# skywoodsz/qm_control

Hardware: NVIDIA H100
Metric: mpc_wbc_iters_per_s (higher is better)
Workload: dtype f64

## Files before the change

qm_control_b200/csrc/capi_mpc.inc:

```

extern "C" {

int qmb200_centroidal_state_from_rbd(const qmb200_handle* h, int32_t n, const double* rbd, double* x) {
  if (!h || !rbd || !x) return -1; const DevModel& d = h->hm.dev;
  for (int r = 0; r < n; ++r) {
    const double* s = rbd + (size_t)r * QMB200_RBD; double* o = x + (size_t)r * NX;
    const double z = s[0], y = s[1], xr = s[2];
    const double sz = sin(z), cz = cos(z), sy = sin(y), cy = cos(y), sx = sin(xr), cx = cos(xr);
    const double R[9] = {cz * cy, cz * sy * sx - sz * cx, cz * sy * cx + sz * sx, sz * cy, sz * sy * sx + cz * cx, sz * sy * cx - cz * sx, -sy, cy * sx, cy * cx};
    const double w[3] = {s[NQ], s[NQ + 1], s[NQ + 2]};
    const double ed[3] = {(cz * sy / cy) * w[0] + (sy * sz / cy) * w[1] + w[2], -sz * w[0] + cz * w[1], (cz / cy) * w[0] + (sz / cy) * w[1]};
    double c[3]; for (int i = 0; i < 3; ++i) c[i] = R[3 * i] * d.c_nom[0] + R[3 * i + 1] * d.c_nom[1] + R[3 * i + 2] * d.c_nom[2];
    const double cw[3] = {c[1] * w[2] - c[2] * w[1], c[2] * w[0] - c[0] * w[2], c[0] * w[1] - c[1] * w[0]};
    double Rtw[3], IRtw[3], L[3];
    for (int i = 0; i < 3; ++i) Rtw[i] = R[i] * w[0] + R[3 + i] * w[1] + R[6 + i] * w[2];
    for (int i = 0; i < 3; ++i) IRtw[i] = d.I_nom[3 * i] * Rtw[0] + d.I_nom[3 * i + 1] * Rtw[1] + d.I_nom[3 * i + 2] * Rtw[2];
    for (int i = 0; i < 3; ++i) L[i] = R[3 * i] * IRtw[0] + R[3 * i + 1] * IRtw[1] + R[3 * i + 2] * IRtw[2];
    (void)ed;
    for (int i = 0; i < 3; ++i) { o[i] = s[NQ + 3 + i] + cw[i]; o[3 + i] = L[i] / d.total_mass; o[6 + i] = s[3 + i]; o[9 + i] = s[i]; }
    for (int j = 0; j < NJ; ++j) o[12 + j] = s[6 + j];
  }
  return 0;
}

// ... 218 lines not shown
int qmb200_set_pipeline(qmb200_handle* h, int chunks) {
  if (!h) return -1; QMB_CUDA(h, cudaSetDevice(h->device));
  if (chunks < 1 || chunks > qmb200_handle::MAX_CHUNKS) return fail(h, "qmb200_set_pipeline: chunks must be in [1, 8]");
  if (chunks > h->B) chunks = h->B;
  if (!h->fork_ev) QMB_CUDA(h, cudaEventCreateWithFlags(&h->fork_ev, cudaEventDisableTiming));
  for (int c = 0; c < chunks; ++c) { if (!h->cs[c]) QMB_CUDA(h, cudaStreamCreateWithFlags(&h->cs[c], cudaStreamNonBlocking)); if (!h->join_ev[c]) QMB_CUDA(h, cudaEventCreateWithFlags(&h->join_ev[c], cudaEventDisableTiming)); }
  h->chunks = chunks; return 0;
}
int qmb200_set_profiling(qmb200_handle* h, int on) {
  if (!h) return -1; QMB_CUDA(h, cudaSetDevice(h->device));
  if (on && !h->ev[0]) for (int i = 0; i < 8; ++i) QMB_CUDA(h, cudaEventCreate(&h->ev[i]));
  h->profiling = on != 0; for (double& v : h->kernel_ms) v = 0.0; h->kernel_calls = 0; h->ev_pending = false; return 0;
}
int qmb200_collect_kernel_times(qmb200_handle* h) {
  if (!h || !h->profiling || !h->ev_pending) return -1; QMB_CUDA(h, cudaSetDevice(h->device)); QMB_CUDA(h, cudaEventSynchronize(h->ev[6]));
  const int a[6] = {0, 1, 2, 3, 4, 5}, b[6] = {1, 2, 3, 4, 5, 6};
  for (int i = 0; i < 6; ++i) { float ms = 0; QMB_CUDA(h, cudaEventElapsedTime(&ms, h->ev[a[i]], h->ev[b[i]])); h->kernel_ms[i] += ms; }
  { float ms = 0; QMB_CUDA(h, cudaEventElapsedTime(&ms, h->ev[1], h->ev[7])); h->kernel_ms[6] += ms; }
  h->kernel_calls += 1; h->ev_pending = false; return 0;
}
int qmb200_get_kernel_times(qmb200_handle* h, double* ms6) { if (!h || !ms6) return -1; for (int i = 0; i < 6; ++i) ms6[i] = h->kernel_calls ? h->kernel_ms[i] / h->kernel_calls : 0.0; return 0; }
int qmb200_get_flow_kernel_time(qmb200_handle* h, double* ms) { if (!h || !ms) return -1; *ms = h->kernel_calls ? h->kernel_ms[6] / h->kernel_calls : 0.0; return 0; }
int qmb200_measure_fp64_peak(qmb200_handle* h, double* tflops) { if (!h || !tflops) return -1; QMB_CUDA(h, cudaSetDevice(h->device)); *tflops = measure_fp64_peak(h->stream); QMB_CUDA(h, cudaGetLastError()); return 0; }

int qmb200_debug_get_step(qmb200_handle* h, double* dx , double* du , double* robot ) {
  if (!h) return -1; QMB_CUDA(h, cudaSetDevice(h->device)); const size_t Bn = (size_t)h->B * h->nmax;
  if (dx) QMB_CUDA(h, cudaMemcpy(dx, h->mpc.dx, Bn * NX * 8, cudaMemcpyDeviceToHost)); if (du) QMB_CUDA(h, cudaMemcpy(du, h->mpc.du, Bn * NU * 8, cudaMemcpyDeviceToHost));
  if (robot) QMB_CUDA(h, cudaMemcpy(robot, h->mpc.robot, (size_t)h->B * ROBOT_DBL * 8, cudaMemcpyDeviceToHost)); return 0;
}

}
```

qm_control_b200/csrc/kernels/mpc_api.cuh:

```cuda
#pragma once
#include <cuda_runtime.h>

#include <string>
#include <vector>

#include "dev_common.cuh"

namespace qmb {

constexpr int EMAX = 32, KMAX = 4, TARGET_DIM = 37;
constexpr int LDX = 36, LDB = 28, LDG = 34, LDH = 24;
constexpr int ST_AR = 0;
constexpr int ST_BR = ST_AR + 9 * LDX;
constexpr int ST_Q = ST_BR + 9 * LDB;
constexpr int Q_PACKED = 480;
__host__ __device__ constexpr int q_row_offset(int r) { return (r & 1) ? 2 * ((r >> 1) + 1) * ((r >> 1) + 1) : 2 * (r >> 1) * ((r >> 1) + 1); }
__host__ __device__ constexpr int q_row_padded(int r) { return (r + 2) & ~1; }
static_assert(q_row_offset(29) + q_row_padded(29) == Q_PACKED && q_row_offset(1) == 2 && q_row_offset(2) == 4 && q_row_offset(3) == 8, "packed lower triangle with even rows");
constexpr int ST_TAIL = ST_Q + Q_PACKED;
constexpr int T_PXJ = 0;
constexpr int T_b = 144, T_q = 174, T_r = 204;
constexpr int T_RT = 222;
constexpr int T_SJ = 276;
constexpr int T_PU2 = 372, T_PED = 380;
// ... 7 lines not shown

struct MpcSolutionDev { int32_t* n_nodes = nullptr; double* t = nullptr; int32_t* event = nullptr; double* x = nullptr; double* u = nullptr; };

struct MpcBuffers {
  int B = 0, nmax = 0, cur = 0;
  double *t0 = nullptr, *x0 = nullptr, *event_times = nullptr, *target_times = nullptr, *target_states = nullptr;
  int32_t *n_events = nullptr, *modes = nullptr, *n_target = nullptr;
  MpcSolutionDev sol[2];
  double *ddp_trial = nullptr;
  double *node_rec = nullptr;
  double *stage = nullptr, *gains = nullptr, *dx = nullptr, *du = nullptr, *robot = nullptr, *step_info = nullptr;
  int32_t *stage_i = nullptr, *status = nullptr;
};
bool mpc_alloc(MpcBuffers& m, int B, int nmax, std::string& err, std::vector<void*>& allocs, cudaStream_t stream);
int mpc_configure_device();

struct MpcProblemDev { const double* t0; const double* x0; const int32_t* n_events; const double* event_times; const int32_t* modes; const int32_t* n_target; const double* target_times; const double* target_states; };

int mpc_solve_launch(const DevModel* mdl, const DevModel& host_mdl, MpcBuffers& m, const MpcProblemDev& p, int b0, int b1, cudaStream_t stream, cudaEvent_t* ev = nullptr);
double measure_fp64_peak(cudaStream_t stream);
int mpc_policy_eval_launch(const MpcBuffers& m, const double* t, double* x_des, double* u_des, int32_t* mode, cudaStream_t stream, int b0 = 0, int b1 = -1);
int mpc_fixup_launch(const MpcBuffers& m, cudaStream_t stream);

}
```

qm_control_b200/csrc/kernels/mpc_kernels.cu:

```cuda
#include <cstdlib>
#include "mpc_api.cuh"
#include "mpc_device.cuh"
#include "node_eval.cuh"
#include "wlinalg.cuh"

namespace qmb {

#ifndef QMB_LQ_WARPS
#define QMB_LQ_WARPS 4
#endif
#ifndef QMB_LQ_MINB
#define QMB_LQ_MINB 4
#endif
constexpr int LQ_WARPS = QMB_LQ_WARPS, LS_WARPS = 4, SETUP_WARPS = 4;
enum { MST_ITER_CAP = 1, MST_OVERFLOW = 2, MST_NAN = 4, MST_NOT_PD = 8, MST_NO_STEP = 16, MST_CONVERGED = 32, MST_NEG_DT = 64 };

__device__ __forceinline__ double interval_start(double t, int ev) { return ev == 2 ? t + WEAK_EPS : t; }
__device__ __forceinline__ double interval_end(double t, int ev) { return ev == 1 ? t - WEAK_EPS : t; }
__device__ __forceinline__ int clamp_events(int ne) { return ne < 0 ? 0 : (ne > EMAX ? EMAX : ne); }
__device__ __forceinline__ int clamp_targets(int nk) { return nk < 1 ? 1 : (nk > KMAX ? KMAX : nk); }
__device__ __forceinline__ int flag_mask(int mode) { int m = 0; for (int i = 0; i < 4; ++i) if (contact_flag(mode, i)) m |= 1 << i; return m; }

struct SetupIdx { int iu, ix; double au, ax; };
__host__ __device__ inline size_t setup_smem_per_warp(int nmax) { return (size_t)nmax * (8 + 8 + 4 + sizeof(SetupIdx) + 4) + 8 * EMAX + 64; }
// ... 391 lines not shown
  if (lane < MU) si[SI_FREE + lane] = (lane < m) ? sm.free_idx[lane] : -1;
  if (lane == 0) { si[SI_TYPE] = 0; si[SI_M] = m; si[SI_NDEP] = ndep; tl[T_MISC] = dtw; tl[T_MISC + 1] = dt * cost_val; tl[T_MISC + 2] = dt * dyn_ss; tl[T_MISC + 3] = dt * eq_ss; }
}

#ifndef QMB_TMA
#define QMB_TMA 1
#endif
constexpr int RIC_THREADS = 128, RIC_NTYPE = 512;
struct RicSmem {
  double P[NX * LDX];
  double A[NX * LDX];
  double W[NX * LDX];
  double Bm[NX * LDB], PB[NX * LDB];
  double G[MU * LDG];
  double H[MU * LDH];
  double Lt[MU * MU];
  alignas(16) double tail[TAIL_DBL];
  double dx[32], dut[32], tmp[32];
  double red[RIC_THREADS / 32][4];
  alignas(8) unsigned long long bar[4];
  int flag; int pad_;
  signed char srow[MU + 2], sfirst[MU + 2];
  unsigned char ntype[RIC_NTYPE];
};
static_assert(sizeof(RicSmem) <= 57344 - 64, "Riccati kernel must keep four CTAs per SM");

__device__ __forceinline__ unsigned smem_u32(const void* p) { return (unsigned)__cvta_generic_to_shared(p); }
__device__ __forceinline__ void mbar_init(unsigned long long* b, unsigned count) { asm volatile("mbarrier.init.shared::cta.b64 [%0], %1;\n" ::"r"(smem_u32(b)), "r"(count) : "memory"); }
__device__ __forceinline__ void mbar_expect_tx(unsigned long long* b, unsigned bytes) { asm volatile("mbarrier.arrive.expect_tx.shared::cta.b64 _, [%0], %1;\n" ::"r"(smem_u32(b)), "r"(bytes) : "memory"); }
__device__ __forceinline__ void mbar_wait(unsigned long long* b, unsigned parity) {
  asm volatile("{\n .reg .pred p;\n WAIT_LOOP:\n mbarrier.try_wait.parity.shared::cta.b64 p, [%0], %1;\n @p bra WAIT_DONE;\n bra WAIT_LOOP;\n WAIT_DONE:\n}\n" ::"r"(smem_u32(b)), "r"(parity) : "memory");
}
__device__ __forceinline__ void bulk_g2s(void* dst, const void* src, unsigned bytes, unsigned long long* bar) {
  asm volatile("cp.async.bulk.shared::cluster.global.mbarrier::complete_tx::bytes [%0], [%1], %2, [%3];\n" ::"r"(smem_u32(dst)), "l"(src), "r"(bytes), "r"(smem_u32(bar)) : "memory");
}
__device__ __forceinline__ void cp_async16(void* smem_dst, const void* gmem_src) { asm volatile("cp.async.cg.shared.global [%0], [%1], 16;\n" ::"r"(smem_u32(smem_dst)), "l"(gmem_src) : "memory"); }
__device__ __forceinline__ void cp_async_wait_all() { asm volatile("cp.async.wait_all;\n" ::: "memory"); }
struct CopyGroup {
  unsigned long long* bar; unsigned phase;
  __device__ __forceinline__ void begin(unsigned bytes, int tid) { if (QMB_TMA && tid == 0) mbar_expect_tx(bar, bytes); }
  __device__ __forceinline__ void copy(void* dst, const void* src, unsigned bytes, int tid, int nthr = RIC_THREADS, int t0 = 0) {
    if (QMB_TMA) { if (tid == 0) bulk_g2s(dst, src, bytes, bar); }
    else { const int me = tid - t0; if (me >= 0 && me < nthr) for (unsigned o = 16u * me; o < bytes; o += 16u * nthr) cp_async16((char*)dst + o, (const char*)src + o); }
  }
  __device__ __forceinline__ void wait() { if (QMB_TMA) mbar_wait(bar, phase & 1u); else { cp_async_wait_all(); __syncthreads(); } ++phase; }
  __device__ __forceinline__ void skip() { ++phase; }
};

// ... 32 lines not shown
    for (int n = 0; n < NT; ++n) { const int ri = i0 + 8 * m + g; if (ri < rows) *reinterpret_cast<double2*>(M + ri * ld + j0 + 8 * n + 2 * t) = make_double2(c[m][n][0], c[m][n][1]); }
}
__device__ __forceinline__ int sup_pos(int j, int first) { return j < 6 ? j : ((j >= 9 && j < 12) ? j - 3 : (((unsigned)(j - 12 - first) < 3u) ? 9 + j - 12 - first : -1)); }

__global__ void __launch_bounds__(RIC_THREADS, 4) mpc_riccati_kernel(const DevModel* __restrict__ mdl, int b0, int B, int nmax, MpcProblemDev p, MpcSolutionDev sol, const double* __restrict__ stage,
                                                                  double* __restrict__ gains, double* __restrict__ dxo, double* __restrict__ duo, double* __restrict__ robot, int32_t* __restrict__ status) {
  extern __shared__ __align__(16) unsigned char smem_raw[];
  RicSmem& sm = *reinterpret_cast<RicSmem*>(smem_raw);
  const int tid = threadIdx.x, warp = tid >> 5, lane = tid & 31, ti = tid >> 2, jb = tid & 3; const int b = b0 + blockIdx.x;
  if (status[b] & MST_CONVERGED) return;
  const int n = sol.n_nodes[b]; const int N = n - 1;
  const double* sgb = stage + (size_t)b * nmax * STAGE_DBL; double* gb = gains + (size_t)b * nmax * GAIN_DBL;
  const int lfp = pack_leg_foot(mdl); const double imass = 1.0 / mdl->total_mass;
  for (int e = tid; e < (int)(sizeof(RicSmem) / 8); e += RIC_THREADS) reinterpret_cast<double*>(&sm)[e] = 0.0;
  __syncthreads();
  if (tid < NX && (tid < 3 || tid >= 24)) sm.A[tid * LDX + tid] = 1.0;
  if (tid == 0) { for (int i = 0; i < 4; ++i) mbar_init(&sm.bar[i], 1); asm volatile("fence.mbarrier_init.release.cluster;\n" ::: "memory"); }
  asm volatile("fence.proxy.async.shared::cta;\n" ::: "memory");
  const bool types_in_smem = n <= RIC_NTYPE;
  auto rec_type = [&](int k) -> int { return reinterpret_cast<const int32_t*>(sgb + (size_t)k * STAGE_DBL + ST_TAIL + T_INT)[SI_TYPE]; };
  if (types_in_smem) for (int k = tid; k < n; k += RIC_THREADS) sm.ntype[k] = (unsigned char)rec_type(k);
  auto node_type = [&](int k) -> int { return types_in_smem ? (int)sm.ntype[k] : rec_type(k); };
  CopyGroup gAB{&sm.bar[0], 0u}, gT{&sm.bar[1], 0u}, gQ{&sm.bar[2], 0u}, gF1{&sm.bar[3], 0u};
  auto issue_ab = [&](int k) { const double* sg = sgb + (size_t)k * STAGE_DBL; gAB.begin((9 * LDX + 9 * LDB) * 8, tid);
    gAB.copy(sm.A + 3 * LDX, sg + ST_AR, 9 * LDX * 8, tid); gAB.copy(sm.Bm + 3 * LDB, sg + ST_BR, 9 * LDB * 8, tid); };
  auto issue_tail = [&](int k) { gT.begin(TAIL_DBL * 8, tid); gT.copy(sm.tail, sgb + (size_t)k * STAGE_DBL + ST_TAIL, TAIL_DBL * 8, tid); };
  auto issue_q = [&](int k) { gQ.begin(Q_PACKED * 8, tid); gQ.copy(sm.Bm, sgb + (size_t)k * STAGE_DBL + ST_Q, Q_PACKED * 8, tid); };
  auto expand = [&]() {
    const double* tl = sm.tail; const int32_t* si = reinterpret_cast<const int32_t*>(tl + T_INT); const double dtw = tl[T_MISC];
    for (int e = tid; e < 144; e += RIC_THREADS) { const int j12 = e / 12, c = e - 12 * j12; const int col = sup_col(c, 3 * (j12 / 3));
      sm.A[(12 + j12) * LDX + col] = ((col == 12 + j12) ? 1.0 : 0.0) + dtw * tl[T_PXJ + e]; }
    if (tid < NX && (tid < 3 || tid >= 12)) sm.A[tid * LDX + NX] = tl[T_b + tid];
    for (int e = tid; e < 21 * MU; e += RIC_THREADS) {
      const int rr = e / MU, a = e - rr * MU; const int r = rr < 3 ? rr : rr + 9; const int fa = si[SI_FREE + a]; double v = 0.0;
      if (fa >= 0) {
        if (r < 3) { if (fa < 12 && fa - 3 * (fa / 3) == r) v = dtw * imass; }
        else if (fa == r) v = dtw;
        else if (fa >= 12 && fa < 24) { const int j = fa - 12, lg = j / 3, foot = (lfp >> (2 * lg)) & 3; const int pv = si[SI_PIV + foot];
          if (pv >= 0 && r == 12 + 3 * lg + pv) { const int jf = j - 3 * lg; v = dtw * tl[T_PU2 + 2 * foot + (jf > pv ? jf - 1 : jf)]; } }
      }
      sm.Bm[r * LDB + a] = v;
    }
    if (tid < MU) { const int fa = si[SI_FREE + tid]; int slot = -1, first = 0;
      if (fa >= 12 && fa < 24) { const int j = fa - 12, lg = j / 3, foot = (lfp >> (2 * lg)) & 3; const int pv = si[SI_PIV + foot]; if (pv >= 0) { const int jf = j - 3 * lg; slot = 2 * foot + (jf > pv ? jf - 1 : jf); first = 3 * lg; } }
      sm.srow[tid] = (signed char)slot; sm.sfirst[tid] = (signed char)first; }
  };
  for (int e = tid; e < NX * NX; e += RIC_THREADS) { const int r = e / NX, c = e - r * NX; sm.P[r * LDX + c] = sgb[(size_t)N * STAGE_DBL + ST_Q + q_row_offset(r > c ? r : c) + (r > c ? c : r)]; }
  if (tid < NX) sm.P[tid * LDX + NX] = sgb[(size_t)N * STAGE_DBL + ST_TAIL + T_q + tid];
  double perf0 = 0, perf1 = 0, perf2 = 0;
  for (int k = tid; k < n; k += RIC_THREADS) { const double* pf = sgb + (size_t)k * STAGE_DBL + ST_TAIL + T_MISC + 1; perf0 += pf[0]; perf1 += pf[1]; perf2 += pf[2]; }
  if (tid < NX) { const double d = p.x0[(size_t)b * NX + tid] - sol.x[(size_t)b * nmax * NX + tid]; sm.dx[tid] = d; perf1 += d * d; }
  perf0 = warp_sum(perf0); perf1 = warp_sum(perf1); perf2 = warp_sum(perf2);
  if (lane == 0) { sm.red[warp][0] = perf0; sm.red[warp][1] = perf1; sm.red[warp][2] = perf2; }
  __syncthreads();
  double perf[3]; for (int i = 0; i < 3; ++i) perf[i] = sm.red[0][i] + sm.red[1][i] + sm.red[2][i] + sm.red[3][i];
  if (N >= 1) { issue_tail(N - 1); if (node_type(N - 1) != 1) issue_ab(N - 1); gT.wait(); if (node_type(N - 1) != 1) expand(); }
  int st = 0;
  const int g = lane >> 2, t = lane & 3;
  for (int k = N - 1; k >= 0; --k) {
    const int type = node_type(k); const int tnext = k > 0 ? node_type(k - 1) : 1;
    if (type == 1) {
      __syncthreads();
      if (tid < NX) { double sv = sm.P[tid * LDX + NX]; for (int j = 0; j < NX; ++j) sv = fma(sm.P[tid * LDX + j], sm.tail[T_b + j], sv); sm.tmp[tid] = sv; }
      __syncthreads();
      if (tid < NX) sm.P[tid * LDX + NX] = sm.tmp[tid];
      if (k > 0) { issue_tail(k - 1); if (tnext != 1) issue_ab(k - 1); gT.wait(); if (tnext != 1) expand(); }
      continue;
    }
    gAB.wait(); if (QMB_TMA) __syncthreads();
    const double dtw_k = sm.tail[T_MISC]; const int acol0 = reinterpret_cast<const int32_t*>(sm.tail + T_INT)[SI_M] - 6;
    { const int i0 = 16 * (warp >> 1), j0 = 16 * (warp & 1);
      double c[2][2][2] = {};
      if (warp & 1) {
#pragma unroll
        for (int m = 0; m < 2; ++m) { const int ri = i0 + 8 * m + g; if (ri < NX) {
            if (t < 3) { c[m][1][0] = sm.P[(24 + 2 * t) * LDX + ri]; c[m][1][1] = sm.P[(25 + 2 * t) * LDX + ri]; }
            else { double sv = sm.P[ri * LDX + NX];
#pragma unroll
              for (int kk = 24; kk < NX; ++kk) sv = fma(sm.P[kk * LDX + ri], sm.A[kk * LDX + NX], sv);
              c[m][1][0] = sv; } } } }
      warp_mma<24, 2, 2, false>(sm.P, LDX, i0, sm.A, LDX, j0, c, g, t);
      cfrag_store<2, 2>(sm.W, LDX, i0, j0, NX, c, g, t);
      double d[1][3][2];
#pragma unroll
      for (int nn = 0; nn < 3; ++nn)
#pragma unroll
        for (int e = 0; e < 2; ++e) { const int a = 8 * nn + 2 * t + e - acol0, ri = 8 * warp + g; d[0][nn][e] = ((unsigned)a < 6u && ri < NX) ? dtw_k * sm.P[(24 + a) * LDX + ri] : 0.0; }
      warp_mma<24, 1, 3, false>(sm.P, LDX, 8 * warp, sm.Bm, LDB, 0, d, g, t);
      cfrag_store<1, 3>(sm.PB, LDB, 8 * warp, 0, NX, d, g, t); }
    __syncthreads();
    if (tid < NX) sm.P[tid * LDX + NX] = sm.tail[T_q + tid];
    { const double* tl = sm.tail; const int32_t* si = reinterpret_cast<const int32_t*>(tl + T_INT); const int mm = si[SI_M];
      double c[3][1][2];
#pragma unroll
      for (int mt = 0; mt < 3; ++mt) { const int a = 8 * mt + g; const bool rowok = a < MU; const int slot = rowok ? sm.srow[a] : -1, first = rowok ? sm.sfirst[a] : 0;
#pragma unroll
        for (int e = 0; e < 2; ++e) { const int j = 8 * warp + 2 * t + e; double v = 0.0;
          if (rowok) { if (j == NX) v = tl[T_r + a]; else if (slot >= 0 && j < NX) { const int ps = sup_pos(j, first); if (ps >= 0) v = tl[T_SJ + slot * 12 + ps]; }
            if ((unsigned)(a - acol0) < 6u) v = fma(dtw_k, sm.W[(24 + a - acol0) * LDX + j], v); }
          c[mt][0][e] = v; } }
      warp_mma<24, 3, 1, false>(sm.Bm, LDB, 0, sm.W, LDX, 8 * warp, c, g, t); cfrag_store<3, 1>(sm.G, LDG, 0, 8 * warp, MU, c, g, t);
      if (warp < 3) { double d[3][1][2];
#pragma unroll
        for (int mt = 0; mt < 3; ++mt) { const int a = 8 * mt + g; const int fa = (a < MU) ? si[SI_FREE + a] : -1;
#pragma unroll
          for (int e = 0; e < 2; ++e) { const int cc = 8 * warp + 2 * t + e; double v = 0.0;
            if (a < MU && cc < MU) { if (a >= mm) v = (a == cc) ? 1.0 : 0.0;
              else if (fa >= 24) v = (a == cc) ? tl[T_RT + 3 * a] : 0.0;
              else { const int fc = si[SI_FREE + cc]; if (fc >= 0 && fc / 3 == fa / 3) v = tl[T_RT + 3 * a + fc - 3 * (fc / 3)]; }
              if ((unsigned)(a - acol0) < 6u) v = fma(dtw_k, sm.PB[(24 + a - acol0) * LDB + cc], v); }
            d[mt][0][e] = v; } }
        warp_mma<24, 3, 1, false>(sm.Bm, LDB, 0, sm.PB, LDB, 8 * warp, d, g, t); cfrag_store<3, 1>(sm.H, LDH, 0, 8 * warp, MU, d, g, t); } }
    __syncthreads();
    issue_q(k);
    if (k > 0) issue_tail(k - 1);
    const int sw = (k + b) & 3;
    if (!QMB_TMA) gQ.wait();
    if (warp == sw) {
      if (QMB_TMA) gQ.skip();
      double hr[MU], y[MU]; double dinv = 0.0; bool ok = true; double* Yb = sm.PB;
#pragma unroll
      for (int c = 0; c < MU; ++c) { hr[c] = (lane < MU) ? sm.H[c * LDH + lane] : 0.0; y[c] = sm.G[c * LDG + lane]; }
#pragma unroll
      for (int j = 0; j < MU; ++j) {
        const double djj = __shfl_sync(FULL, hr[j], j); if (!(djj > 0.0)) ok = false;
        const double inv = rsqrt(djj); const double lij = hr[j] * inv;
        if (lane == j) dinv = inv;
        if (lane < MU) sm.Lt[j * MU + lane] = lij;
        y[j] *= inv; Yb[j * LDX + lane] = y[j];
#pragma unroll
        for (int c = j + 1; c < MU; ++c) { const double lcj = __shfl_sync(FULL, lij, c); hr[c] = fma(-lij, lcj, hr[c]); y[c] = fma(-lcj, y[j], y[c]); }
      }
      if (lane < MU) sm.dut[lane] = dinv;
      if (!ok && lane == 0) sm.flag = 1;
      __syncwarp();
      double* gk = gb + (size_t)k * GAIN_DBL;
#pragma unroll
      for (int a = MU - 1; a >= 0; --a) {
        asm volatile("" ::: "memory");
        y[a] *= sm.dut[a];
        gk[a * LDG + lane] = -y[a];
#pragma unroll
        for (int c = 0; c < a; ++c) y[c] = fma(-sm.Lt[c * MU + a], y[a], y[c]);
      }
    } else {
      if (QMB_TMA) gQ.wait();
      const int hi = (warp - sw - 1) & 3;
      for (int tile = hi; tile < 16; tile += 3) { const int i0 = 8 * (tile >> 2), j0 = 8 * (tile & 3);
        double c[1][1][2]; const int ri = i0 + g;
#pragma unroll
        for (int e = 0; e < 2; ++e) { const int cj = j0 + 2 * t + e; double v = (ri < NX && cj <= NX) ? (cj == NX ? sm.P[ri * LDX + NX] : (cj <= ri ? sm.Bm[q_row_offset(ri) + cj] : sm.Bm[q_row_offset(cj) + ri])) : 0.0;
          if (ri >= 24 && ri < NX && cj <= NX) v += sm.W[ri * LDX + cj];
          c[0][0][e] = v; }
        warp_mma<24, 1, 1, false>(sm.A, LDX, i0, sm.W, LDX, j0, c, g, t); cfrag_store<1, 1>(sm.P, LDX, i0, j0, NX, c, g, t); }
    }
    __syncthreads();
    if (sm.flag) { st |= MST_NOT_PD; if (k > 0) gT.wait(); break; }
    if (k > 0) { if (tnext != 1) issue_ab(k - 1); gT.wait(); if (tnext != 1) expand(); }
    { const double* Yb = sm.PB; const int i0 = 16 * (warp >> 1), j0 = 16 * (warp & 1);
      double c[2][2][2]; cfrag_load<2, 2>(sm.P, LDX, i0, j0, NX, c, g, t); warp_mma<MU, 2, 2, true>(Yb, LDX, i0, Yb, LDX, j0, c, g, t); cfrag_store<2, 2>(sm.P, LDX, i0, j0, NX, c, g, t); }
  }
  __syncthreads();
  double armijo = 0.0, dxn2 = 0.0, dun2 = 0.0;
  if (!(st & MST_NOT_PD)) {
    auto issue_fwd = [&](int k) {
      if (k >= N) return; const int o = k & 1; CopyGroup& cg = o ? gF1 : gAB; const double* sg = sgb + (size_t)k * STAGE_DBL; const bool ev = node_type(k) == 1;
      cg.begin((ev ? 0 : (GAIN_DBL + 9 * LDX + 9 * LDB) * 8) + TAIL_DBL * 8, tid);
      cg.copy((o ? sm.P : sm.A) + 9 * LDX, sg + ST_TAIL, TAIL_DBL * 8, tid);
      if (!ev) { cg.copy(o ? sm.W : sm.G, gb + (size_t)k * GAIN_DBL, GAIN_DBL * 8, tid); cg.copy(o ? sm.P : sm.A, sg + ST_AR, 9 * LDX * 8, tid); cg.copy(o ? sm.PB : sm.Bm, sg + ST_BR, 9 * LDB * 8, tid); } };
    issue_fwd(0);
    for (int k = 0; k < N; ++k) {
      const int o = k & 1; const double* Kb = o ? sm.W : sm.G; const double* ARb = o ? sm.P : sm.A; const double* BRb = o ? sm.PB : sm.Bm; const double* tl = (o ? sm.P : sm.A) + 9 * LDX;
      double* dxk = dxo + ((size_t)b * nmax + k) * NX; double* duk = duo + ((size_t)b * nmax + k) * NU;
      const double* dxc = (k & 1) ? sm.tmp : sm.dx; double* dxn = (k & 1) ? sm.dx : sm.tmp;
      if (o) gF1.wait(); else gAB.wait();
      if (QMB_TMA) __syncthreads();
      issue_fwd(k + 1);
      const int32_t* si = reinterpret_cast<const int32_t*>(tl + T_INT); const int type = si[SI_TYPE], ndep = si[SI_NDEP], mm = si[SI_M]; const double dtw = tl[T_MISC];
      if (tid < NX) { const double dxi = dxc[tid]; dxk[tid] = dxi; dxn2 += dxi * dxi; }
      if (type == 1) { if (tid < NX) { duk[tid] = 0.0; dxn[tid] = dxc[tid] + tl[T_b + tid]; } continue; }
      { double s = 0.0;
        if (ti < MU) { const double* kr = Kb + ti * LDG + jb * 8; const double* dx = dxc + jb * 8;
#pragma unroll
          for (int v = 0; v < 8; ++v) s = fma(kr[v], dx[v], s); }
        s += __shfl_xor_sync(FULL, s, 1); s += __shfl_xor_sync(FULL, s, 2); if (ti < MU && jb == 0) sm.dut[ti] = s + Kb[ti * LDG + NX]; }
// ... 1 lines not shown
      {
        static_assert(MAXDEP * 8 == RIC_THREADS, "one 8-thread group per dependent input");
        const int d = tid >> 3, q8 = tid & 7; double s = 0.0; const int di = (d < ndep) ? si[SI_DEP + d] : -1;
        if (di >= 12) { const int j = di - 12, lg = j / 3, first = 3 * lg; const double* px = tl + T_PXJ + j * 12;
          s = px[q8] * dxc[sup_col(q8, first)]; if (q8 < 4) s = fma(px[q8 + 8], dxc[sup_col(q8 + 8, first)], s);
          if (q8 >= 4 && q8 < 6) { const int foot = (lfp >> (2 * lg)) & 3; const int col = si[SI_PCOL + 2 * foot + q8 - 4]; if (si[SI_PIV + foot] >= 0 && col >= 0) s = fma(tl[T_PU2 + 2 * foot + q8 - 4], sm.dut[col], s); } }
        s += __shfl_xor_sync(FULL, s, 1); s += __shfl_xor_sync(FULL, s, 2); s += __shfl_xor_sync(FULL, s, 4);
        if (di >= 0 && q8 == 0) { const double full = s + tl[T_PED + d]; duk[di] = full; dun2 += full * full; if (di >= 12) dxn[di] = dxc[di] + dtw * s + tl[T_b + di]; } }
      if (tid < NX) armijo += tl[T_q + tid] * dxc[tid];
      if (tid < MU) { const double dut = sm.dut[tid]; armijo += tl[T_r + tid] * dut; const int fi = si[SI_FREE + tid];
        if (fi >= 0) { duk[fi] = dut; dun2 += dut * dut; if (fi >= 12) dxn[fi] = dxc[fi] + dtw * dut + tl[T_b + fi]; } }
      if (warp == 1 && lane < 3) { double acc = 0.0; for (int a = 0; a < mm; ++a) { const int fa = si[SI_FREE + a]; if (fa < 12 && fa - 3 * (fa / 3) == lane) acc += sm.dut[a]; }
        dxn[lane] = dxc[lane] + dtw * imass * acc + tl[T_b + lane]; }
      if (warp >= 2) { const int rr = (tid - 64) >> 2; double s = 0.0;
        if (rr < 9) { const double* ar = ARb + rr * LDX + jb * 8; const double* dx = dxc + jb * 8;
#pragma unroll
          for (int v = 0; v < 8; ++v) s = fma(ar[v], dx[v], s);
          if (jb < 3) { const double* br = BRb + rr * LDB + jb * 8; const double* du = sm.dut + jb * 8;
#pragma unroll
            for (int v = 0; v < 8; ++v) s = fma(br[v], du[v], s); } }
        s += __shfl_xor_sync(FULL, s, 1); s += __shfl_xor_sync(FULL, s, 2); if (rr < 9 && jb == 0) dxn[3 + rr] = s + tl[T_b + 3 + rr]; }
    }
    __syncthreads();
    if (tid < NX) { const double dxi = ((N & 1) ? sm.tmp : sm.dx)[tid]; dxo[((size_t)b * nmax + N) * NX + tid] = dxi; duo[((size_t)b * nmax + N) * NU + tid] = 0.0; dxn2 += dxi * dxi; armijo += sgb[(size_t)N * STAGE_DBL + ST_TAIL + T_q + tid] * dxi; }
  }
  armijo = warp_sum(armijo); dxn2 = warp_sum(dxn2); dun2 = warp_sum(dun2);
  __syncthreads();
  if (lane == 0) { sm.red[warp][0] = armijo; sm.red[warp][1] = dxn2; sm.red[warp][2] = dun2; }
  __syncthreads();
  if (tid == 0) { double a = 0, x2 = 0, u2 = 0; for (int w = 0; w < RIC_THREADS / 32; ++w) { a += sm.red[w][0]; x2 += sm.red[w][1]; u2 += sm.red[w][2]; }
    double* rb = robot + (size_t)b * ROBOT_DBL; rb[0] = a; rb[1] = perf[0]; rb[2] = perf[1]; rb[3] = perf[2]; rb[4] = sqrt(x2); rb[5] = sqrt(u2); if (st) atomicOr(&status[b], st); }
}

__device__ __forceinline__ void fixup_inputs(MpcSolutionDev sol, int b, int nmax, int n, int tid, int nthreads) {
  const int32_t* ge = sol.event + (size_t)b * nmax; double* gu = sol.u + (size_t)b * nmax * NU;
  for (int i = tid; i < NU; i += nthreads) for (int k = 1; k < n; ++k) if ((k == n - 1) || (ge[k] == 1)) gu[(size_t)k * NU + i] = gu[(size_t)(k - 1) * NU + i];
}

#ifndef QMB_LS_MINB
#define QMB_LS_MINB 4
#endif
__global__ void __launch_bounds__(32 * LS_WARPS, QMB_LS_MINB) mpc_linesearch_kernel(const DevModel* __restrict__ mdl, int b0, int B, int nmax, MpcProblemDev p, MpcSolutionDev sol, const double* __restrict__ dxo, const double* __restrict__ duo,
                                                                     const double* __restrict__ robot, int32_t* __restrict__ status, double* __restrict__ step_info, int iteration) {
  __shared__ double red[LS_WARPS][3]; __shared__ int decision; __shared__ double s_ev[EMAX]; __shared__ unsigned char s_modes[EMAX + 8];
  const int tid = threadIdx.x, warp = tid >> 5, lane = tid & 31; const int b = b0 + blockIdx.x; if (b >= B) return;
  if (status[b] & MST_CONVERGED) return;
  const int n = sol.n_nodes[b]; const int N = n - 1;
  const double* gt = sol.t + (size_t)b * nmax; const int32_t* ge = sol.event + (size_t)b * nmax;
  double* gx = sol.x + (size_t)b * nmax * NX; double* gu = sol.u + (size_t)b * nmax * NU; const double* gdx = dxo + (size_t)b * nmax * NX; const double* gdu = duo + (size_t)b * nmax * NU;
// ... 279 lines not shown
  for (int it = 0; it < iters; ++it) {
    mpc_flow_kernel<<<(unsigned)((nodes + 32 * FL_WARPS - 1) / (32 * FL_WARPS)), 32 * FL_WARPS, FL_SMEM, stream>>>(mdl, b0, b1, nmax, p, next, m.node_rec, m.status);
    if (ev && it == iters - 1) cudaEventRecord(ev[7], stream);
    mpc_lq_kernel<<<(unsigned)((nodes + LQ_WARPS - 1) / LQ_WARPS), 32 * LQ_WARPS, sizeof(LqSmem) * LQ_WARPS, stream>>>(mdl, b0, b1, nmax, p, next, m.node_rec, m.stage, m.status);
    if (ev && it == iters - 1) cudaEventRecord(ev[2], stream);
    mpc_riccati_kernel<<<nb, RIC_THREADS, sizeof(RicSmem), stream>>>(mdl, b0, b1, nmax, p, next, m.stage, m.gains, m.dx, m.du, m.robot, m.status);
    if (ev && it == iters - 1) cudaEventRecord(ev[3], stream);
    if (ddp) { mpc_rollout_trials_kernel<<<(nb + ro_rpc - 1) / ro_rpc, ro_rpc * tr_pitch, (size_t)ro_rpc * GAIN_DBL * 8, stream>>>(mdl, b0, b1, nmax, p, next, m.stage, m.gains, m.ddp_trial, m.robot, m.status, n_trials, tr_pitch, ro_rpc);
      mpc_rollout_kernel<<<ro_grid, RO_THREADS, 0, stream>>>(mdl, b0, b1, nmax, p, next, m.stage, m.gains, m.ddp_trial, m.robot, m.status, m.step_info, 2, n_trials, tr_pitch, it); ++launched; }
    else mpc_linesearch_kernel<<<nb, 32 * LS_WARPS, 0, stream>>>(mdl, b0, b1, nmax, p, next, m.dx, m.du, m.robot, m.status, m.step_info, it);
    launched += 4;
  }
  if (ev) cudaEventRecord(ev[4], stream);
  return launched;
}

int mpc_policy_eval_launch(const MpcBuffers& m, const double* t, double* x_des, double* u_des, int32_t* mode, cudaStream_t stream, int b0, int b1) {
  if (b1 < 0) b1 = m.B; if (b1 <= b0) return 0;
  mpc_policy_eval_kernel<<<(b1 - b0 + 3) / 4, 128, 0, stream>>>(b0, b1, m.nmax, m.sol[m.cur], m.n_events, m.event_times, m.modes, t, x_des, u_des, mode);
  return 1;
}
int mpc_fixup_launch(const MpcBuffers& m, cudaStream_t stream) { mpc_fixup_kernel<<<m.B, 32, 0, stream>>>(m.B, m.nmax, m.sol[m.cur]); return 1; }

__global__ void __launch_bounds__(256) fp64_peak_kernel(double* out, int iters, double a, double b) {
  double x0 = threadIdx.x, x1 = x0 + 1, x2 = x0 + 2, x3 = x0 + 3, x4 = x0 + 4, x5 = x0 + 5, x6 = x0 + 6, x7 = x0 + 7;
  for (int i = 0; i < iters; ++i) { x0 = fma(x0, a, b); x1 = fma(x1, a, b); x2 = fma(x2, a, b); x3 = fma(x3, a, b); x4 = fma(x4, a, b); x5 = fma(x5, a, b); x6 = fma(x6, a, b); x7 = fma(x7, a, b); }
  if (x0 + x1 + x2 + x3 + x4 + x5 + x6 + x7 == 12345.678) out[0] = x0;
}
double measure_fp64_peak(cudaStream_t stream) {
  double* d = nullptr; cudaMalloc(&d, 8); cudaEvent_t e0, e1; cudaEventCreate(&e0); cudaEventCreate(&e1);
  int dev = 0, sms = 132; cudaGetDevice(&dev); cudaDeviceGetAttribute(&sms, cudaDevAttrMultiProcessorCount, dev);
  const int blocks = sms * 8, iters = 1 << 15; double best = 0.0;
  fp64_peak_kernel<<<blocks, 256, 0, stream>>>(d, 1024, 0.999999, 1e-9);
  for (int rep = 0; rep < 3; ++rep) {
    cudaEventRecord(e0, stream); fp64_peak_kernel<<<blocks, 256, 0, stream>>>(d, iters, 0.999999, 1e-9); cudaEventRecord(e1, stream); cudaEventSynchronize(e1);
    float ms = 0; cudaEventElapsedTime(&ms, e0, e1); const double tf = 2.0 * 8.0 * iters * 256.0 * blocks / (ms * 1e-3) / 1e12; if (tf > best) best = tf;
  }
  cudaEventDestroy(e0); cudaEventDestroy(e1); cudaFree(d); return best;
}

}
```

qm_control_b200/interface.py:

```python
import ctypes as C
import os

import numpy as np

from . import _lib
from ._lib import NX, NU, RBD, CMD, TARGET, EMAX, KMAX, Config, QmbError, dp, ip


class QMInterface:
    def __init__(self, taskFile=None, urdfFile=None, referenceFile=None, wbcGainsFile=None):
        self.taskFile = taskFile or _lib.asset("qm_task.info")
        self.urdfFile = urdfFile or _lib.asset("qm_robot.urdf")
        self.referenceFile = referenceFile or _lib.asset("qm_reference.info")
        self.gaitFile = _lib.asset("qm_gait.info")
        self.wbcGainsFile = wbcGainsFile
        for what, path in (("Task file", self.taskFile), ("URDF file", self.urdfFile), ("targetCommand file", self.referenceFile)):
            if not os.path.exists(path):
                raise ValueError("[QMInterface] %s not found: %s" % (what, path))


def _f64(a, shape=None):
    a = np.ascontiguousarray(a, dtype=np.float64)
    if shape is not None and tuple(a.shape) != tuple(shape):
        raise ValueError("expected shape %s, got %s" % (shape, a.shape))
# ... 181 lines not shown
        rc = self.lib.qmb200_gait_bin_permutation(n, _p(_f64(prob["t0"])), _p(_i32(prob["n_events"])), _p(_f64(prob["event_times"])), _p(_i32(prob["modes"])), _p(perm))
        if rc != 0:
            raise QmbError("qmb200_gait_bin_permutation failed")
        return perm

    def set_pipeline(self, chunks):
        self._chk(self.lib.qmb200_set_pipeline(self.h, int(chunks)), "qmb200_set_pipeline")

    def set_profiling(self, on=True):
        self._chk(self.lib.qmb200_set_profiling(self.h, 1 if on else 0), "qmb200_set_profiling")

    def collect_kernel_times(self):
        self.lib.qmb200_collect_kernel_times(self.h)

    def kernel_times(self):
        ms = np.zeros(6); self._chk(self.lib.qmb200_get_kernel_times(self.h, _p(ms)), "qmb200_get_kernel_times")
        d = dict(zip(("setup", "lq", "riccati", "linesearch", "policy_eval", "wbc"), ms.tolist()))
        v = C.c_double(); self._chk(self.lib.qmb200_get_flow_kernel_time(self.h, C.byref(v)), "qmb200_get_flow_kernel_time"); d["lq_flow"] = v.value
        return d

    def measure_fp64_peak(self):
        v = C.c_double(); self._chk(self.lib.qmb200_measure_fp64_peak(self.h, C.byref(v)), "qmb200_measure_fp64_peak"); return v.value

    def debug_get_step(self):
        B, N = self.batch, self.nmax; dx = np.zeros((B, N, NX)); du = np.zeros((B, N, NU)); robot = np.zeros((B, 8))
        self._chk(self.lib.qmb200_debug_get_step(self.h, _p(dx), _p(du), _p(robot)), "qmb200_debug_get_step"); return dx, du, robot

    def observation_update(self, rbd, period, t_obs, x_obs):
        B = self.batch; rbd = _f64(rbd, (B, RBD)); period = _f64(period, (B,)); t = _f64(t_obs, (B,)).copy(); x = _f64(x_obs, (B, NX)).copy()
        self._chk(self.lib.qmb200_observation_update(self.h, _p(rbd), _p(period), _p(t), _p(x)), "qmb200_observation_update"); return t, x

    def target_trajectories(self, kind, cmd, t_obs, x_obs, ee_state, last_ee_target):
        B = self.batch; c = np.zeros((B, 7)); cmd = np.asarray(cmd, dtype=np.float64).reshape(B, -1); c[:, :cmd.shape[1]] = cmd
        t = _f64(t_obs, (B,)); x = _f64(x_obs, (B, NX)); ee = _f64(ee_state, (B, 7)); le = _f64(last_ee_target, (B, 7)).copy()
        nt = np.zeros(B, dtype=np.int32); tt = np.zeros((B, KMAX)); ts = np.zeros((B, KMAX, TARGET))
        self._chk(self.lib.qmb200_target_trajectories(self.h, int(kind), _p(c), _p(t), _p(x), _p(ee), _p(le), _p(nt), _p(tt), _p(ts)), "qmb200_target_trajectories"); return nt, tt, ts, le

    def initial_ee_target(self):
        v = np.zeros(7); self.lib.qmb200_initial_ee_target(_p(v)); return np.tile(v, (self.batch, 1))

    def set_arm_gains(self, kp, kd):
        self._chk(self.lib.qmb200_set_arm_gains(self.h, float(kp), float(kd)), "qmb200_set_arm_gains")

    def control_law(self, x_des, u_des, wbc_cmd, t_obs, x_obs, joint_cmd, arm_pos_cmd, last_time):
        B = self.batch; jc = _f64(joint_cmd, (B, 18, 5)).copy(); ap = _f64(arm_pos_cmd, (B, 6)).copy(); lt = _f64(last_time, (B,)).copy(); st = np.zeros(B, dtype=np.int32)
        self._chk(self.lib.qmb200_control_law(self.h, _p(_f64(x_des, (B, NX))), _p(_f64(u_des, (B, NU))), _p(_f64(wbc_cmd, (B, CMD))), _p(_f64(t_obs, (B,))), _p(_f64(x_obs, (B, NX))), _p(jc), _p(ap), _p(lt), _p(st)),
# ... 54 lines not shown
```

Baseline: 19.37.

## Overlap next-stage A/B load and expansion with serial Cholesky in Riccati

In the TMA path, the three helper warps now synchronise on a named barrier after their phase-3 work. They then issue the next node's A/B copy and run the tail expansion, all while the designated warp runs the serial factorisation, rather than doing this after the block-wide barrier. The serial warp waits on the tail copy itself. This aims to hide per-node load and expand latency in the backward Riccati sweep, at the cost of a more intricate sync order and a changed abort path on non-PD. Optional clock64 per-phase profiling counters are also added behind a compile flag, off by default.

```diff
diff --git a/qm_control_b200/csrc/capi_mpc.inc b/qm_control_b200/csrc/capi_mpc.inc
--- a/qm_control_b200/csrc/capi_mpc.inc
+++ b/qm_control_b200/csrc/capi_mpc.inc
@@ -264,6 +264,12 @@
 int qmb200_get_kernel_times(qmb200_handle* h, double* ms6) { if (!h || !ms6) return -1; for (int i = 0; i < 6; ++i) ms6[i] = h->kernel_calls ? h->kernel_ms[i] / h->kernel_calls : 0.0; return 0; }
 int qmb200_get_flow_kernel_time(qmb200_handle* h, double* ms) { if (!h || !ms) return -1; *ms = h->kernel_calls ? h->kernel_ms[6] / h->kernel_calls : 0.0; return 0; }
 int qmb200_measure_fp64_peak(qmb200_handle* h, double* tflops) { if (!h || !tflops) return -1; QMB_CUDA(h, cudaSetDevice(h->device)); *tflops = measure_fp64_peak(h->stream); QMB_CUDA(h, cudaGetLastError()); return 0; }
+#if QMB_RIC_PROF
+int qmb200_ric_profile(qmb200_handle* h, unsigned long long* counters, int n, int reset) {
+  if (!h || !counters) return -1; QMB_CUDA(h, cudaSetDevice(h->device)); QMB_CUDA(h, cudaStreamSynchronize(h->stream));
+  const int got = ric_prof_read(counters, n, reset != 0); if (got < 0) return fail(h, "qmb200_ric_profile: counter copy failed"); return got;
+}
+#endif
 
 int qmb200_debug_get_step(qmb200_handle* h, double* dx , double* du , double* robot ) {
   if (!h) return -1; QMB_CUDA(h, cudaSetDevice(h->device)); const size_t Bn = (size_t)h->B * h->nmax;
diff --git a/qm_control_b200/csrc/kernels/mpc_api.cuh b/qm_control_b200/csrc/kernels/mpc_api.cuh
--- a/qm_control_b200/csrc/kernels/mpc_api.cuh
+++ b/qm_control_b200/csrc/kernels/mpc_api.cuh
@@ -53,4 +53,12 @@
 int mpc_policy_eval_launch(const MpcBuffers& m, const double* t, double* x_des, double* u_des, int32_t* mode, cudaStream_t stream, int b0 = 0, int b1 = -1);
 int mpc_fixup_launch(const MpcBuffers& m, cudaStream_t stream);
 
+#ifndef QMB_RIC_PROF
+#define QMB_RIC_PROF 0
+#endif
+enum RicProfSlot { RP_WAIT = 0, RP_PH1, RP_PH2, RP_PH3_SERIAL, RP_PH3_HELPER, RP_PH3_BARRIER, RP_TAIL, RP_PH4, RP_FWD, RP_NODES, RP_CTAS, RP_NSLOT };
+#if QMB_RIC_PROF
+int ric_prof_read(unsigned long long* out, int n, bool reset);
+#endif
+
 }
diff --git a/qm_control_b200/csrc/kernels/mpc_kernels.cu b/qm_control_b200/csrc/kernels/mpc_kernels.cu
--- a/qm_control_b200/csrc/kernels/mpc_kernels.cu
+++ b/qm_control_b200/csrc/kernels/mpc_kernels.cu
@@ -437,8 +437,26 @@
   int flag; int pad_;
   signed char srow[MU + 2], sfirst[MU + 2];
   unsigned char ntype[RIC_NTYPE];
+#if QMB_RIC_PROF
+  unsigned long long prof[RIC_THREADS / 32][RP_NSLOT];
+#endif
 };
 static_assert(sizeof(RicSmem) <= 57344 - 64, "Riccati kernel must keep four CTAs per SM");
+
+#if QMB_RIC_PROF
+__device__ unsigned long long g_ric_prof[RP_NSLOT];
+#define RIC_PROF_START long long ric_t0 = clock64()
+#define RIC_MARK(s) do { if (lane == 0) { const long long ric_now = clock64(); sm.prof[warp][(s)] += (unsigned long long)(ric_now - ric_t0); ric_t0 = ric_now; } } while (0)
+#define RIC_SKIP() do { if (lane == 0) ric_t0 = clock64(); } while (0)
+#define RIC_COUNT(s) do { if (lane == 0) sm.prof[warp][(s)] += 1ull; } while (0)
+#define RIC_PROF_FLUSH() do { if (lane == 0) for (int s_ = 0; s_ < RP_NSLOT; ++s_) atomicAdd(&g_ric_prof[s_], sm.prof[warp][s_]); } while (0)
+#else
+#define RIC_PROF_START
+#define RIC_MARK(s) ((void)0)
+#define RIC_SKIP() ((void)0)
+#define RIC_COUNT(s) ((void)0)
+#define RIC_PROF_FLUSH() ((void)0)
+#endif
 
 __device__ __forceinline__ unsigned smem_u32(const void* p) { return (unsigned)__cvta_generic_to_shared(p); }
 __device__ __forceinline__ void mbar_init(unsigned long long* b, unsigned count) { asm volatile("mbarrier.init.shared::cta.b64 [%0], %1;\n" ::"r"(smem_u32(b)), "r"(count) : "memory"); }
@@ -517,16 +535,17 @@
   if (types_in_smem) for (int k = tid; k < n; k += RIC_THREADS) sm.ntype[k] = (unsigned char)rec_type(k);
   auto node_type = [&](int k) -> int { return types_in_smem ? (int)sm.ntype[k] : rec_type(k); };
   CopyGroup gAB{&sm.bar[0], 0u}, gT{&sm.bar[1], 0u}, gQ{&sm.bar[2], 0u}, gF1{&sm.bar[3], 0u};
-  auto issue_ab = [&](int k) { const double* sg = sgb + (size_t)k * STAGE_DBL; gAB.begin((9 * LDX + 9 * LDB) * 8, tid);
-    gAB.copy(sm.A + 3 * LDX, sg + ST_AR, 9 * LDX * 8, tid); gAB.copy(sm.Bm + 3 * LDB, sg + ST_BR, 9 * LDB * 8, tid); };
+  auto issue_ab = [&](int k, int me = -1) { if (me < 0) me = tid; const double* sg = sgb + (size_t)k * STAGE_DBL; gAB.begin((9 * LDX + 9 * LDB) * 8, me);
+    gAB.copy(sm.A + 3 * LDX, sg + ST_AR, 9 * LDX * 8, me); gAB.copy(sm.Bm + 3 * LDB, sg + ST_BR, 9 * LDB * 8, me); };
   auto issue_tail = [&](int k) { gT.begin(TAIL_DBL * 8, tid); gT.copy(sm.tail, sgb + (size_t)k * STAGE_DBL + ST_TAIL, TAIL_DBL * 8, tid); };
   auto issue_q = [&](int k) { gQ.begin(Q_PACKED * 8, tid); gQ.copy(sm.Bm, sgb + (size_t)k * STAGE_DBL + ST_Q, Q_PACKED * 8, tid); };
-  auto expand = [&]() {
+  auto expand = [&](int me = -1, int nthr = RIC_THREADS) {
+    if (me < 0) me = tid;
     const double* tl = sm.tail; const int32_t* si = reinterpret_cast<const int32_t*>(tl + T_INT); const double dtw = tl[T_MISC];
-    for (int e = tid; e < 144; e += RIC_THREADS) { const int j12 = e / 12, c = e - 12 * j12; const int col = sup_col(c, 3 * (j12 / 3));
+    for (int e = me; e < 144; e += nthr) { const int j12 = e / 12, c = e - 12 * j12; const int col = sup_col(c, 3 * (j12 / 3));
       sm.A[(12 + j12) * LDX + col] = ((col == 12 + j12) ? 1.0 : 0.0) + dtw * tl[T_PXJ + e]; }
-    if (tid < NX && (tid < 3 || tid >= 12)) sm.A[tid * LDX + NX] = tl[T_b + tid];
-    for (int e = tid; e < 21 * MU; e += RIC_THREADS) {
+    if (me < NX && (me < 3 || me >= 12)) sm.A[me * LDX + NX] = tl[T_b + me];
+    for (int e = me; e < 21 * MU; e += nthr) {
       const int rr = e / MU, a = e - rr * MU; const int r = rr < 3 ? rr : rr + 9; const int fa = si[SI_FREE + a]; double v = 0.0;
       if (fa >= 0) {
         if (r < 3) { if (fa < 12 && fa - 3 * (fa / 3) == r) v = dtw * imass; }
@@ -536,9 +555,9 @@
       }
       sm.Bm[r * LDB + a] = v;
     }
-    if (tid < MU) { const int fa = si[SI_FREE + tid]; int slot = -1, first = 0;
+    if (me < MU) { const int fa = si[SI_FREE + me]; int slot = -1, first = 0;
       if (fa >= 12 && fa < 24) { const int j = fa - 12, lg = j / 3, foot = (lfp >> (2 * lg)) & 3; const int pv = si[SI_PIV + foot]; if (pv >= 0) { const int jf = j - 3 * lg; slot = 2 * foot + (jf > pv ? jf - 1 : jf); first = 3 * lg; } }
-      sm.srow[tid] = (signed char)slot; sm.sfirst[tid] = (signed char)first; }
+      sm.srow[me] = (signed char)slot; sm.sfirst[me] = (signed char)first; }
   };
   for (int e = tid; e < NX * NX; e += RIC_THREADS) { const int r = e / NX, c = e - r * NX; sm.P[r * LDX + c] = sgb[(size_t)N * STAGE_DBL + ST_Q + q_row_offset(r > c ? r : c) + (r > c ? c : r)]; }
   if (tid < NX) sm.P[tid * LDX + NX] = sgb[(size_t)N * STAGE_DBL + ST_TAIL + T_q + tid];
@@ -552,6 +571,7 @@
   if (N >= 1) { issue_tail(N - 1); if (node_type(N - 1) != 1) issue_ab(N - 1); gT.wait(); if (node_type(N - 1) != 1) expand(); }
   int st = 0;
   const int g = lane >> 2, t = lane & 3;
+  RIC_PROF_START; RIC_COUNT(RP_CTAS);
   for (int k = N - 1; k >= 0; --k) {
     const int type = node_type(k); const int tnext = k > 0 ? node_type(k - 1) : 1;
     if (type == 1) {
@@ -560,9 +580,11 @@
       __syncthreads();
       if (tid < NX) sm.P[tid * LDX + NX] = sm.tmp[tid];
       if (k > 0) { issue_tail(k - 1); if (tnext != 1) issue_ab(k - 1); gT.wait(); if (tnext != 1) expand(); }
+      RIC_SKIP();
       continue;
     }
     gAB.wait(); if (QMB_TMA) __syncthreads();
+    RIC_MARK(RP_WAIT); RIC_COUNT(RP_NODES);
     const double dtw_k = sm.tail[T_MISC]; const int acol0 = reinterpret_cast<const int32_t*>(sm.tail + T_INT)[SI_M] - 6;
     { const int i0 = 16 * (warp >> 1), j0 = 16 * (warp & 1);
       double c[2][2][2] = {};
@@ -584,6 +606,7 @@
       warp_mma<24, 1, 3, false>(sm.P, LDX, 8 * warp, sm.Bm, LDB, 0, d, g, t);
       cfrag_store<1, 3>(sm.PB, LDB, 8 * warp, 0, NX, d, g, t); }
     __syncthreads();
+    RIC_MARK(RP_PH1);
     if (tid < NX) sm.P[tid * LDX + NX] = sm.tail[T_q + tid];
     { const double* tl = sm.tail; const int32_t* si = reinterpret_cast<const int32_t*>(tl + T_INT); const int mm = si[SI_M];
       double c[3][1][2];
@@ -609,6 +632,7 @@
     __syncthreads();
     issue_q(k);
     if (k > 0) issue_tail(k - 1);
+    RIC_MARK(RP_PH2);
     const int sw = (k + b) & 3;
     if (!QMB_TMA) gQ.wait();
     if (warp == sw) {
@@ -638,6 +662,8 @@
 #pragma unroll
         for (int c = 0; c < a; ++c) y[c] = fma(-sm.Lt[c * MU + a], y[a], y[c]);
       }
+      RIC_MARK(RP_PH3_SERIAL);
+      if (QMB_TMA && k > 0) gT.wait();
     } else {
       if (QMB_TMA) gQ.wait();
       const int hi = (warp - sw - 1) & 3;
@@ -648,14 +674,28 @@
           if (ri >= 24 && ri < NX && cj <= NX) v += sm.W[ri * LDX + cj];
           c[0][0][e] = v; }
         warp_mma<24, 1, 1, false>(sm.A, LDX, i0, sm.W, LDX, j0, c, g, t); cfrag_store<1, 1>(sm.P, LDX, i0, j0, NX, c, g, t); }
+      RIC_MARK(RP_PH3_HELPER);
+      if (QMB_TMA && k > 0) {
+        asm volatile("bar.sync 1, 96;\n" ::: "memory");
+        const int me = 32 * hi + lane;
+        if (tnext != 1) issue_ab(k - 1, me);
+        gT.wait(); if (tnext != 1) expand(me, 96);
+        RIC_MARK(RP_TAIL);
+      }
     }
     __syncthreads();
-    if (sm.flag) { st |= MST_NOT_PD; if (k > 0) gT.wait(); break; }
-    if (k > 0) { if (tnext != 1) issue_ab(k - 1); gT.wait(); if (tnext != 1) expand(); }
+    RIC_MARK(RP_PH3_BARRIER);
+    if (sm.flag) { st |= MST_NOT_PD;
+      if (QMB_TMA) { if (k > 0 && tnext != 1) gAB.wait(); } else if (k > 0) gT.wait();
+      break; }
+    if (!QMB_TMA && k > 0) { if (tnext != 1) issue_ab(k - 1); gT.wait(); if (tnext != 1) expand(); }
+    RIC_MARK(RP_TAIL);
     { const double* Yb = sm.PB; const int i0 = 16 * (warp >> 1), j0 = 16 * (warp & 1);
       double c[2][2][2]; cfrag_load<2, 2>(sm.P, LDX, i0, j0, NX, c, g, t); warp_mma<MU, 2, 2, true>(Yb, LDX, i0, Yb, LDX, j0, c, g, t); cfrag_store<2, 2>(sm.P, LDX, i0, j0, NX, c, g, t); }
+    RIC_MARK(RP_PH4);
   }
   __syncthreads();
+  RIC_SKIP();
   double armijo = 0.0, dxn2 = 0.0, dun2 = 0.0;
   if (!(st & MST_NOT_PD)) {
     auto issue_fwd = [&](int k) {
@@ -703,9 +743,11 @@
         s += __shfl_xor_sync(FULL, s, 1); s += __shfl_xor_sync(FULL, s, 2); if (rr < 9 && jb == 0) dxn[3 + rr] = s + tl[T_b + 3 + rr]; }
     }
     __syncthreads();
+    RIC_MARK(RP_FWD);
     if (tid < NX) { const double dxi = ((N & 1) ? sm.tmp : sm.dx)[tid]; dxo[((size_t)b * nmax + N) * NX + tid] = dxi; duo[((size_t)b * nmax + N) * NU + tid] = 0.0; dxn2 += dxi * dxi; armijo += sgb[(size_t)N * STAGE_DBL + ST_TAIL + T_q + tid] * dxi; }
   }
   armijo = warp_sum(armijo); dxn2 = warp_sum(dxn2); dun2 = warp_sum(dun2);
+  RIC_PROF_FLUSH();
   __syncthreads();
   if (lane == 0) { sm.red[warp][0] = armijo; sm.red[warp][1] = dxn2; sm.red[warp][2] = dun2; }
   __syncthreads();
@@ -1031,6 +1073,15 @@
 }
 int mpc_fixup_launch(const MpcBuffers& m, cudaStream_t stream) { mpc_fixup_kernel<<<m.B, 32, 0, stream>>>(m.B, m.nmax, m.sol[m.cur]); return 1; }
 
+#if QMB_RIC_PROF
+int ric_prof_read(unsigned long long* out, int n, bool reset) {
+  n = n < RP_NSLOT ? n : RP_NSLOT; if (n <= 0) return 0;
+  if (cudaMemcpyFromSymbol(out, g_ric_prof, n * sizeof(unsigned long long)) != cudaSuccess) return -1;
+  if (reset) { const unsigned long long zero[RP_NSLOT] = {}; if (cudaMemcpyToSymbol(g_ric_prof, zero, sizeof(zero)) != cudaSuccess) return -1; }
+  return n;
+}
+#endif
+
 __global__ void __launch_bounds__(256) fp64_peak_kernel(double* out, int iters, double a, double b) {
   double x0 = threadIdx.x, x1 = x0 + 1, x2 = x0 + 2, x3 = x0 + 3, x4 = x0 + 4, x5 = x0 + 5, x6 = x0 + 6, x7 = x0 + 7;
   for (int i = 0; i < iters; ++i) { x0 = fma(x0, a, b); x1 = fma(x1, a, b); x2 = fma(x2, a, b); x3 = fma(x3, a, b); x4 = fma(x4, a, b); x5 = fma(x5, a, b); x6 = fma(x6, a, b); x7 = fma(x7, a, b); }
diff --git a/qm_control_b200/interface.py b/qm_control_b200/interface.py
--- a/qm_control_b200/interface.py
+++ b/qm_control_b200/interface.py
@@ -227,6 +227,18 @@
     def measure_fp64_peak(self):
         v = C.c_double(); self._chk(self.lib.qmb200_measure_fp64_peak(self.h, C.byref(v)), "qmb200_measure_fp64_peak"); return v.value
 
+    RIC_PROF_SLOTS = ("wait", "phase1", "phase2", "phase3_serial", "phase3_helper", "phase3_barrier", "tail", "phase4", "forward", "nodes", "ctas")
+
+    def ric_profile(self, reset=True):
+        fn = getattr(self.lib, "qmb200_ric_profile", None)
+        if fn is None:
+            raise QmbError("this libqmb200.so was built without -DQMB_RIC_PROF=1 (tools/build_variants.sh prof=\"-DQMB_RIC_PROF=1\")")
+        v = np.zeros(len(self.RIC_PROF_SLOTS), dtype=np.uint64)
+        n = fn(self.h, _p(v), C.c_int(len(v)), C.c_int(1 if reset else 0))
+        if n != len(v):
+            raise QmbError("qmb200_ric_profile failed: %s" % self.lib.qmb200_last_error(self.h))
+        return dict(zip(self.RIC_PROF_SLOTS, (int(x) for x in v)))
+
     def debug_get_step(self):
         B, N = self.batch, self.nmax; dx = np.zeros((B, N, NX)); du = np.zeros((B, N, NU)); robot = np.zeros((B, 8))
         self._chk(self.lib.qmb200_debug_get_step(self.h, _p(dx), _p(du), _p(robot)), "qmb200_debug_get_step"); return dx, du, robot
```

After: 19.79 (median of 6 runs). +2.2%, better.
